# KTH-RPL/HiMo

Measured on AMD Instinct MI355X. Metric: lidar_frames_per_sec_120k, higher is better.
Workload: dtype f16x2 (two-term split fp16, x = h + l with exact subnormals, on the matrix cores; float32 accumulate; ~22-bit products); 1 GPU; per-frame pipeline: pillarise 3 sweeps (512x512 grid) -> SeFlow++-style encoder/decoder + GRU head (random-init, self-specified: reference network source absent) -> per-point flow -> ego-motion removal + dt0 + flow2compDis -> comp_dis; points_per_frame=120000, sweeps_per_frame=3, parallelism=frames sharded x1, refined_output=False, batches_in_flight=3, matrix_arithmetic=f16x2, samples_per_backbone_launch=16, collectives=none (single process)

## Files before the change

himo_amd/csrc/conv_common.h:

```cpp
#pragma once
#include "himo_common.h"
#include "bf16x3.h"
#include <math.h>

namespace himo {

typedef float floatx16 __attribute__((ext_vector_type(16)));

enum Epilogue {
    kEpiBias = 0,
    kEpiBiasBnGelu = 1,
    kEpiBiasGelu = 2,
    kEpiGruZR = 3,
    kEpiGruQ = 4,
    kEpiBiasRelu = 5,
    kEpiReluMask = 6
};

struct ConvArgs {
    const float* x; int64_t x_batch_stride; int x_pitch;
    const float* w;
    const float* bias; const float* scale; const float* shift;
    float* y; int64_t y_batch_stride; int y_pitch;
    int N, H, W, Cin, Cout;
    int n_inner; int64_t x_outer_stride, y_outer_stride;
    int Ho, Wo;
    const float* aux_in; int aux_in_pitch;
    float* aux_out; int aux_out_pitch;
    int act_flags;
    unsigned* range_seen;
    const unsigned long long* mask;
    int64_t mask_batch_stride, mask_outer_stride;
};
enum ActFlags { kActSplitIn = 1, kActSplitOut = 2, kActVecStore = 4, kActAccumulate = 8, kActStuffedIn = 16, kActRowMask = 32 };

__device__ inline int64_t image_offset(int img, int n_inner, int64_t batch_stride, int64_t outer_stride) {
    return (int64_t)(img % n_inner) * batch_stride + (int64_t)(img / n_inner) * outer_stride;
}

__device__ inline int xcd_block_id(int bid, int n_blocks) {
    const int per = n_blocks >> 3, rem = n_blocks & 7;
    const int xcd = bid & 7, idx = bid >> 3;
    return xcd * per + (xcd < rem ? xcd : rem) + idx;
}

__device__ inline float gelu_exact(float v) {
    const float hv = 0.5f * v;
    const float t = __builtin_amdgcn_rcpf(fmaf(0.3275911f * 0.70710678118654752440f, fabsf(v), 1.0f));
    float p = fmaf(1.061405429f, t, -1.453152027f);
    p = fmaf(p, t, 1.421413741f);
    p = fmaf(p, t, -0.284496736f);
    p = fmaf(p, t, 0.254829592f);
    const float ex = __builtin_amdgcn_exp2f((v * v) * (-0.5f * 1.44269504088896340736f));
    const float e = fmaf(-(p * t), ex, 1.0f);
    return fmaf(fabsf(hv), e, hv);
}
__device__ inline float gelu_grad_exact(float v) {
    const float t = __builtin_amdgcn_rcpf(fmaf(0.3275911f * 0.70710678118654752440f, fabsf(v), 1.0f));
    float p = fmaf(1.061405429f, t, -1.453152027f);
    p = fmaf(p, t, 1.421413741f);
    p = fmaf(p, t, -0.284496736f);
    p = fmaf(p, t, 0.254829592f);
    const float ex = __builtin_amdgcn_exp2f((v * v) * (-0.5f * 1.44269504088896340736f));
    const float e = fmaf(-(p * t), ex, 1.0f);
    return fmaf(v * 0.39894228040143267794f, ex, 0.5f + copysignf(0.5f * e, v));
}
__device__ inline float sigmoid_f(float v) { return __builtin_amdgcn_rcpf(1.0f + __expf(-v)); }
__device__ inline float tanh_f(float v) {
    const float e = __expf(-2.0f * fabsf(v));
    const float t = (1.0f - e) * __builtin_amdgcn_rcpf(1.0f + e);
    return copysignf(t, v);
}


template <int EPI> constexpr bool kEpiAffine = EPI == kEpiBias || EPI == kEpiBiasBnGelu || EPI == kEpiBiasGelu;
template <int EPI>
__device__ inline void epi_affine(float k, float bias, float sc, float sh, float& A, float& B) {
    if (EPI == kEpiBiasBnGelu) { A = k * sc; B = fmaf(bias, sc, sh); } else { A = k; B = bias; }
}
template <int EPI>
__device__ inline float epi_activate(float acc, float A, float B) {
    const float v = fmaf(acc, A, B);
    return EPI == kEpiBias ? v : gelu_exact(v);
}

template <int EPI>
__device__ inline void epilogue_store(const ConvArgs& a, float* __restrict__ yout, int64_t pix, int co, float v, float sc, float sh) {
    if (EPI == kEpiBias) {
        yout[pix * a.y_pitch + co] = v;
    } else if (EPI == kEpiBiasBnGelu) {
        v = v * sc + sh;
        yout[pix * a.y_pitch + co] = gelu_exact(v);
    } else if (EPI == kEpiBiasGelu) {
        yout[pix * a.y_pitch + co] = gelu_exact(v);
    } else if (EPI == kEpiGruZR) {
        const int half = a.Cout / 2;
        const float g = sigmoid_f(v);
        if (co < half) yout[pix * a.y_pitch + co] = g;
        else a.aux_out[pix * a.aux_out_pitch + (co - half)] = g * a.aux_in[pix * a.aux_in_pitch + (co - half)];
    } else if (EPI == kEpiBiasRelu) {
        yout[pix * a.y_pitch + co] = fmaxf(v, 0.f);
    } else if (EPI == kEpiReluMask) {
        yout[pix * a.y_pitch + co] = a.aux_in[pix * a.aux_in_pitch + co] > 0.f ? v : 0.f;
    } else if (EPI == kEpiGruQ) {
        const float q = tanh_f(v);
        const float z = a.aux_in[pix * a.aux_in_pitch + co];
        const float h = a.aux_out[pix * a.aux_out_pitch + co];
        a.aux_out[pix * a.aux_out_pitch + co] = (1.0f - z) * h + z * q;
    }
}

__device__ inline unsigned split_word(float v, bool odd);
template <int EPI, bool PAIRED>
__device__ inline void split_store(const ConvArgs& a, float* __restrict__ yout, int64_t pix, int co, float v, float sc, float sh) {
    if (EPI == kEpiBiasBnGelu) v = gelu_exact(v * sc + sh);
    else if (EPI == kEpiBiasGelu) v = gelu_exact(v);
    else if (EPI == kEpiBiasRelu) v = fmaxf(v, 0.f);
    if (PAIRED) {
        const bool odd = co & 1;
        unsigned* rec = reinterpret_cast<unsigned*>(yout + pix * a.y_pitch + (co & ~15));
        rec[(odd ? 8 : 0) + ((co & 15) >> 1)] = split_word(v, odd);
        return;
    }
    unsigned h, l;
    split2_rounded(v, h, l);
    {
        unsigned short* rec = reinterpret_cast<unsigned short*>(yout + pix * a.y_pitch + (co & ~15));
        rec[co & 15] = (unsigned short)h;
        rec[16 + (co & 15)] = (unsigned short)l;
    }
}

constexpr float kSplitRangeGuard = 0.015625f;
__device__ inline void note_range(const ConvArgs& a, float v) {
    if (a.range_seen && __ballot(fabsf(v) >= kSplitRangeGuard) != 0ull && (threadIdx.x & 63) == 0 &&
        __hip_atomic_load(a.range_seen, __ATOMIC_RELAXED, __HIP_MEMORY_SCOPE_AGENT) == 0u)
        __hip_atomic_store(a.range_seen, 1u, __ATOMIC_RELAXED, __HIP_MEMORY_SCOPE_AGENT);
}

inline bool vec_store_ok(const ConvArgs& a) {
    return (reinterpret_cast<uintptr_t>(a.y) & 15u) == 0 && !(a.y_pitch & 3) && !(a.y_batch_stride & 3) && !(a.y_outer_stride & 3) && !(a.Cout & 3) &&
           (int64_t)a.Ho * a.Wo * a.y_pitch < ((int64_t)1 << 29);
}

template <bool OSPLIT, bool MASK = false, bool ACC = false>
__device__ inline void store_block_vec(const ConvArgs& a, float* __restrict__ yout, unsigned char* stg, const unsigned (&word)[16],
                                       int lane, int64_t pix0, int n_valid_px, int ch0) {
    const int li = lane & 31, lh = lane >> 5;
    const int widx = OSPLIT ? (li >> 4) * 16 + ((li & 1) ? 8 : 0) + ((li & 15) >> 1) : li;
#pragma unroll
    for (int r = 0; r < 16; ++r) {
        const int px = (r & 3) + 8 * (r >> 2) + 4 * lh;
        const int slot = px ^ ((px >> 2) & 1);
        *reinterpret_cast<unsigned*>(stg + slot * 128 + widx * 4) = word[r];
    }
    __builtin_amdgcn_wave_barrier();
#pragma unroll
    for (int t = 0; t < 4; ++t) {
        const int q = t * 64 + lane;
        const int slot = q >> 3, piece = q & 7;
        const int px = slot ^ ((slot >> 2) & 1);
        uint4 d = *reinterpret_cast<const uint4*>(stg + q * 16);
        const int ch = ch0 + (OSPLIT ? (piece >> 2) * 16 : piece * 4);
        if (px < n_valid_px && ch < a.Cout) {
            if (MASK) {
                const float4 m = *reinterpret_cast<const float4*>(a.aux_in + (pix0 + px) * (int64_t)a.aux_in_pitch + ch0 + piece * 4);
                d.x = m.x > 0.f ? d.x : 0u; d.y = m.y > 0.f ? d.y : 0u; d.z = m.z > 0.f ? d.z : 0u; d.w = m.w > 0.f ? d.w : 0u;
            }
            float* dst = yout + (((unsigned)pix0 + (unsigned)px) * (unsigned)a.y_pitch + (unsigned)(ch0 + piece * 4));
            if (ACC) {
                const float4 o = *reinterpret_cast<const float4*>(dst);
                d.x = __builtin_bit_cast(unsigned, o.x + __builtin_bit_cast(float, d.x)); d.y = __builtin_bit_cast(unsigned, o.y + __builtin_bit_cast(float, d.y));
                d.z = __builtin_bit_cast(unsigned, o.z + __builtin_bit_cast(float, d.z)); d.w = __builtin_bit_cast(unsigned, o.w + __builtin_bit_cast(float, d.w));
            }
            *reinterpret_cast<uint4*>(dst) = d;
        }
    }
    __builtin_amdgcn_wave_barrier();
}

template <int EPI>
__device__ inline float epilogue_value(float v, float sc, float sh) {
    if (EPI == kEpiBiasBnGelu) return gelu_exact(v * sc + sh);
    if (EPI == kEpiBiasGelu) return gelu_exact(v);
    if (EPI == kEpiBiasRelu) return fmaxf(v, 0.f);
    return v;
}
__device__ inline unsigned split_word(float v, bool odd) {
    const unsigned p = split2_packed(v);
    const unsigned q = (unsigned)__builtin_amdgcn_mov_dpp((int)p, 0xB1, 0xF, 0xF, true);
    return __builtin_amdgcn_perm(q, p, odd ? 0x03020706u : 0x05040100u);
}

}
```

himo_amd/csrc/gruhead.hip:

```cpp
#include "conv_common.h"
#include "bf16x3.h"

namespace himo {

struct GruHeadArgs {
    int64_t n;
    const int* pid; const float* offsets;
    const float* img0; const float* img1; int img_pitch;
    const float* dec; int dec_pitch;
    const float* w_off; const float* b_off;
    const unsigned short* wzr; const float* bzr;
    const unsigned short* wq; const float* bq;
    const unsigned short* w1; const float* b1;
    const float* w2; const float* b2;
    const float* xyz_t; const float* pts; int stride;
    float* flow;
    int iters;
    int img_split;
    unsigned* nonfinite;
    int w2_pitch;
};

constexpr int kGhMaxIters = 4;
struct GruHeadSave {
    float* hx;
    float* rhx;
    float* z; float* r; float* q;
    float* pre1; float* y1;
    float* res;
    int64_t rows;
};

constexpr int kGhMaxSamples = 16;
struct GruHeadSample {
    int64_t n;
    const int* pid; const float* offsets; const float* img0; const float* img1; const float* dec;
    const float* xyz_t; const float* pts; float* flow; int stride;
};
struct GruHeadBatch {
    int n_samples;
    int block_start[kGhMaxSamples + 1];
    GruHeadSample s[kGhMaxSamples];
};

constexpr int kGhRows = 64;
constexpr bool kGhLaunder = false;

template <int SLABS>
__device__ inline int a_slot(int s, int slab, int row, int half) {
    return ((s * SLABS + slab) * kGhRows + row) * 32 + ((half ^ ((row >> 4) & 1)) << 4);
}

template <int FMT, int SLABS>
__device__ inline void a_store(unsigned char* A, int row, int k, float v) {
    constexpr int kGhPlane = SLABS * kGhRows * 32;
    unsigned h, m = 0, l;
    if (FMT == 3) split3(v, h, m, l); else split2(v, h, l);
    const int slab = k >> 4, kk = k & 15;
    const int off = a_slot<SLABS>(0, slab, row, kk >> 3) + (kk & 7) * 2;
    *reinterpret_cast<unsigned short*>(A + off) = (unsigned short)h;
    if (FMT == 3) *reinterpret_cast<unsigned short*>(A + off + kGhPlane) = (unsigned short)m;
    *reinterpret_cast<unsigned short*>(A + off + (FMT - 1) * kGhPlane) = (unsigned short)l;
}

template <int RT, int NT, int FMT, int SLABS>
__device__ inline void gemm192(const unsigned char* A, const unsigned short* __restrict__ wpk, int cout, const int (&col)[NT],
                               floatx16 (&acc)[RT][NT], int rt0, int li, int lh) {
    uint4 bcur[NT][FMT], bnxt[NT][FMT];
    auto load_b = [&](int slab, uint4 (&b)[NT][FMT]) {
#pragma unroll
        for (int t = 0; t < NT; ++t)
#pragma unroll
            for (int s = 0; s < FMT; ++s)
                b[t][s] = *reinterpret_cast<const uint4*>(wpk + (((int64_t)slab * FMT + s) * cout + col[t] + li) * 16 + lh * 8);
    };
    load_b(0, bcur);
    constexpr int kUnroll = SLABS % 2 == 0 ? 2 : 3;
#pragma unroll kUnroll
    for (int slab = 0; slab < SLABS; ++slab) {
        if (slab + 1 < SLABS) load_b(slab + 1, bnxt);
        bf16x8 af[RT][FMT];
#pragma unroll
        for (int rt = 0; rt < RT; ++rt)
#pragma unroll
            for (int s = 0; s < FMT; ++s)
                af[rt][s] = *reinterpret_cast<const bf16x8*>(A + a_slot<SLABS>(s, slab, (rt0 + rt) * 32 + li, lh));
#define HIMO_TERM(SA, SB)                                                                                          \
    _Pragma("unroll") for (int rt = 0; rt < RT; ++rt) _Pragma("unroll") for (int t = 0; t < NT; ++t)                  \
        acc[rt][t] = __builtin_amdgcn_mfma_f32_32x32x16_bf16(af[rt][SA], __builtin_bit_cast(bf16x8, bcur[t][SB]), acc[rt][t], 0, 0, 0);
#define HIMO_TERM16(ACC, SA, SB)                                                                                   \
    _Pragma("unroll") for (int rt = 0; rt < RT; ++rt) _Pragma("unroll") for (int t = 0; t < NT; ++t)                  \
        ACC[rt][t] = __builtin_amdgcn_mfma_f32_32x32x16_f16(__builtin_bit_cast(f16x8, af[rt][SA]),                    \
                                                           __builtin_bit_cast(f16x8, bcur[t][SB]), ACC[rt][t], 0, 0, 0);
        if constexpr (FMT == 3) {
            HIMO_TERM(2, 0) HIMO_TERM(0, 2) HIMO_TERM(1, 1) HIMO_TERM(1, 0) HIMO_TERM(0, 1) HIMO_TERM(0, 0)
        } else {
            HIMO_TERM16(acc, 1, 0) HIMO_TERM16(acc, 0, 1) HIMO_TERM16(acc, 0, 0)
        }
#undef HIMO_TERM16
#undef HIMO_TERM
#pragma unroll
        for (int t = 0; t < NT; ++t)
#pragma unroll
            for (int s = 0; s < FMT; ++s) bcur[t][s] = bnxt[t][s];
    }
    if (FMT == 2) {
#pragma unroll
        for (int rt = 0; rt < RT; ++rt)
#pragma unroll
            for (int t = 0; t < NT; ++t)
#pragma unroll
                for (int r = 0; r < 16; ++r)
                    acc[rt][t][r] = acc[rt][t][r] * kF16AccScale;
    }
}

template <int GROUP>
__device__ inline void sv_store(float* base, unsigned byte_off, float v) {
    *reinterpret_cast<float*>(reinterpret_cast<char*>(base) + byte_off) = v;
}

template <int FMT, int SLABS, bool SAVE = false>
__global__ __launch_bounds__(256, (FMT == 2 && !SAVE) ? 3 : 2) void gru_head_kernel(GruHeadArgs a, GruHeadBatch batch, GruHeadSave sv) {
    constexpr bool FOLD = SLABS == 9;
    static_assert(!(SAVE && FOLD), "the training forward keeps x explicit");
    constexpr int kGhPlane = SLABS * kGhRows * 32;
    __shared__ __attribute__((aligned(16))) unsigned char A[FMT * kGhPlane];
    __shared__ int s_pid[kGhRows];
    const int wave = __builtin_amdgcn_readfirstlane(threadIdx.x >> 6), lane = threadIdx.x & 63;
    const int li = lane & 31, lh = lane >> 5;
    int bid = blockIdx.x;
    {
        int smp = 0;
        while (smp + 1 < batch.n_samples && bid >= batch.block_start[smp + 1]) ++smp;
        bid -= batch.block_start[smp];
        const GruHeadSample& g = batch.s[smp];
        a.n = g.n; a.pid = g.pid; a.offsets = g.offsets; a.img0 = g.img0; a.img1 = g.img1; a.dec = g.dec;
        a.xyz_t = g.xyz_t; a.pts = g.pts; a.flow = g.flow; a.stride = g.stride;
    }
    const int64_t r0 = (int64_t)bid * kGhRows;

    if (threadIdx.x < kGhRows) {
        const int64_t i = r0 + threadIdx.x;
        s_pid[threadIdx.x] = i < a.n ? a.pid[i] : -1;
    }
    if constexpr (FOLD) {
        const int row = threadIdx.x >> 2, q = threadIdx.x & 3;
        const int64_t i = r0 + row;
        float v[4] = {0.f, 0.f, 0.f, 0.f};
        if (q == 0) {
            if (i < a.n) { v[0] = a.offsets[i * 3]; v[1] = a.offsets[i * 3 + 1]; v[2] = a.offsets[i * 3 + 2]; }
            v[3] = 1.f;
        }
#pragma unroll
        for (int k = 0; k < 4; ++k) a_store<FMT, SLABS>(A, row, 128 + q * 4 + k, v[k]);
    } else if constexpr (SAVE) {
        const int c = threadIdx.x & 63;
        const float w0 = a.w_off[c], w1 = a.w_off[64 + c], w2 = a.w_off[128 + c], bc = a.b_off[c];
#pragma unroll 4
        for (int j = 0; j < 16; ++j) {
            const int row = wave + 4 * j;
            const int64_t i = r0 + row;
            const int64_t ic = i < a.n ? i : a.n - 1;
            const float o0 = a.offsets[ic * 3], o1 = a.offsets[ic * 3 + 1], o2 = a.offsets[ic * 3 + 2];
            const float v = fmaf(o2, w2, fmaf(o1, w1, o0 * w0)) + bc;
            a_store<FMT, SLABS>(A, row, 128 + c, v);
            const unsigned at = ((unsigned)i * 192u + 128u + (unsigned)c) * 4u;
            for (int t = 0; t <= a.iters; ++t) sv_store<0>(sv.hx + t * sv.rows * 192, at, v);
            for (int t = 0; t < a.iters; ++t) sv_store<0>(sv.rhx + t * sv.rows * 192, at, v);
        }
    } else {
        const int row = threadIdx.x >> 2, q = threadIdx.x & 3;
        const int64_t i = r0 + row;
        float o0 = 0.f, o1 = 0.f, o2 = 0.f;
        if (i < a.n) { o0 = a.offsets[i * 3]; o1 = a.offsets[i * 3 + 1]; o2 = a.offsets[i * 3 + 2]; }
#pragma unroll
        for (int k = 0; k < 16; ++k) {
            const int c = q * 16 + k;
            const float v = fmaf(o2, a.w_off[128 + c], fmaf(o1, a.w_off[64 + c], o0 * a.w_off[c])) + a.b_off[c];
            a_store<FMT, SLABS>(A, row, 128 + c, v);
        }
    }
    __syncthreads();

    const float* src = wave == 0 ? a.img0 : wave == 1 ? a.img1 : a.dec + (wave - 2) * 32;
    const int src_pitch = wave < 2 ? a.img_pitch : a.dec_pitch;
    float h[2][16];
    {
        int cell[2][16];
#pragma unroll
        for (int rt = 0; rt < 2; ++rt)
#pragma unroll
            for (int r = 0; r < 16; ++r) cell[rt][r] = s_pid[rt * 32 + (r & 3) + 8 * (r >> 2) + 4 * lh];
        if (FMT == 2 && wave < 2 && a.img_split) {
            unsigned short hh[2][16], ll[2][16];
#pragma unroll
            for (int rt = 0; rt < 2; ++rt)
#pragma unroll
                for (int r = 0; r < 16; ++r) {
                    const unsigned short* rec = reinterpret_cast<const unsigned short*>(src + (int64_t)max(cell[rt][r], 0) * src_pitch + (li & ~15));
                    hh[rt][r] = rec[li & 15]; ll[rt][r] = rec[16 + (li & 15)];
                }
#pragma unroll
            for (int rt = 0; rt < 2; ++rt)
#pragma unroll
                for (int r = 0; r < 16; ++r)
                    h[rt][r] = cell[rt][r] >= 0 ? (float)__builtin_bit_cast(_Float16, hh[rt][r]) + (float)__builtin_bit_cast(_Float16, ll[rt][r]) : 0.f;
        } else {
#pragma unroll
            for (int rt = 0; rt < 2; ++rt)
#pragma unroll
                for (int r = 0; r < 16; ++r) h[rt][r] = src[(int64_t)max(cell[rt][r], 0) * src_pitch + li];
#pragma unroll
            for (int rt = 0; rt < 2; ++rt)
#pragma unroll
                for (int r = 0; r < 16; ++r) h[rt][r] = cell[rt][r] >= 0 ? h[rt][r] : 0.f;
            if (FMT == 2 && wave < 2) {
#pragma unroll
                for (int rt = 0; rt < 2; ++rt)
#pragma unroll
                    for (int r = 0; r < 16; ++r) {
                        unsigned hh, ll;
                        split2(h[rt][r], hh, ll);
                        h[rt][r] = (float)__builtin_bit_cast(_Float16, (unsigned short)hh) + (float)__builtin_bit_cast(_Float16, (unsigned short)ll);
                    }
            }
        }
#pragma unroll
        for (int rt = 0; rt < 2; ++rt)
#pragma unroll
            for (int r = 0; r < 16; ++r) {
                const int row = rt * 32 + (r & 3) + 8 * (r >> 2) + 4 * lh;
                a_store<FMT, SLABS>(A, row, wave * 32 + li, h[rt][r]);
                if constexpr (SAVE) sv_store<1>(sv.hx, (((unsigned)r0 + row) * 192u + wave * 32 + li) * 4u, h[rt][r]);
            }
    }
    __syncthreads();
    unsigned o128 = (((unsigned)r0 + 4 * lh) * 128u + wave * 32 + li) * 4u, o192 = (((unsigned)r0 + 4 * lh) * 192u + wave * 32 + li) * 4u;

    const int col_zr[2] = {wave * 32, 128 + wave * 32};
    const int col_q[1] = {wave * 32};
    const float bz = a.bzr[wave * 32 + li], br = a.bzr[128 + wave * 32 + li], bq = a.bq[wave * 32 + li];

#pragma unroll 1
    for (int it = 0; it < a.iters; ++it) {
        int sli = li, slh = lh;
        if constexpr (SAVE || kGhLaunder) asm volatile("" : "+v"(o128), "+v"(o192), "+v"(sli), "+v"(slh));
        float* const sz = SAVE ? sv.z + it * sv.rows * 128 : nullptr; float* const sr = SAVE ? sv.r + it * sv.rows * 128 : nullptr;
        float* const sq = SAVE ? sv.q + it * sv.rows * 128 : nullptr; float* const srhx = SAVE ? sv.rhx + it * sv.rows * 192 : nullptr;
        float* const shx = SAVE ? sv.hx + (it + 1) * sv.rows * 192 : nullptr;
        floatx16 acc[2][2];
#pragma unroll
        for (int rt = 0; rt < 2; ++rt)
#pragma unroll
            for (int t = 0; t < 2; ++t)
#pragma unroll
                for (int r = 0; r < 16; ++r) acc[rt][t][r] = 0.f;
        gemm192<2, 2, FMT, SLABS>(A, a.wzr, 256, col_zr, acc, 0, li, lh);
        __syncthreads();
#pragma unroll
        for (int rt = 0; rt < 2; ++rt)
#pragma unroll
            for (int r = 0; r < 16; ++r) {
                acc[rt][0][r] = sigmoid_f(acc[rt][0][r] + bz);
                const float rr = sigmoid_f(acc[rt][1][r] + br);
                const int row = rt * 32 + (r & 3) + 8 * (r >> 2) + 4 * slh;
                a_store<FMT, SLABS>(A, row, wave * 32 + sli, rr * h[rt][r]);
                if constexpr (SAVE) {
                    const unsigned dr = rt * 32 + (r & 3) + 8 * (r >> 2);
                    sv_store<2>(sz, o128 + dr * 512u, acc[rt][0][r]); sv_store<2>(sr, o128 + dr * 512u, rr);
                    sv_store<3>(srhx, o192 + dr * 768u, rr * h[rt][r]);
                }
            }
        __syncthreads();
        if constexpr (SAVE || kGhLaunder) asm volatile("" : "+v"(o128), "+v"(o192), "+v"(sli), "+v"(slh));
        floatx16 acq[2][1];
#pragma unroll
        for (int rt = 0; rt < 2; ++rt)
#pragma unroll
            for (int r = 0; r < 16; ++r) acq[rt][0][r] = 0.f;
        gemm192<2, 1, FMT, SLABS>(A, a.wq, 128, col_q, acq, 0, li, lh);
        __syncthreads();
#pragma unroll
        for (int rt = 0; rt < 2; ++rt)
#pragma unroll
            for (int r = 0; r < 16; ++r) {
                const float q = tanh_f(acq[rt][0][r] + bq);
                const float zz = acc[rt][0][r];
                const float hn = (1.0f - zz) * h[rt][r] + zz * q;
                h[rt][r] = hn;
                const int row = rt * 32 + (r & 3) + 8 * (r >> 2) + 4 * slh;
                a_store<FMT, SLABS>(A, row, wave * 32 + sli, hn);
                if constexpr (SAVE) {
                    const unsigned dr = rt * 32 + (r & 3) + 8 * (r >> 2);
                    sv_store<4>(sq, o128 + dr * 512u, q);
                    sv_store<5>(shx, o192 + dr * 768u, hn);
                }
            }
        __syncthreads();
    }

    floatx16 ac1[1][1];
#pragma unroll
    for (int r = 0; r < 16; ++r) ac1[0][0][r] = 0.f;
    const int col_1[1] = {0};
    if (wave < 2) gemm192<1, 1, FMT, SLABS>(A, a.w1, 32, col_1, ac1, wave, li, lh);
    __syncthreads();
    float* Y = reinterpret_cast<float*>(A);
    if (wave < 2) {
        const float b1 = a.b1[li];
#pragma unroll
        for (int r = 0; r < 16; ++r) {
            const int row = wave * 32 + (r & 3) + 8 * (r >> 2) + 4 * lh;
            const float pre = ac1[0][0][r] + b1, y = gelu_exact(pre);
            Y[row * 32 + li] = y;
            if constexpr (SAVE) {
                const unsigned at = (((unsigned)r0 + row) * 32u + li) * 4u;
                sv_store<6>(sv.pre1, at, pre); sv_store<6>(sv.y1, at, y);
            }
        }
    }
    __syncthreads();
    if constexpr (SAVE) {
        const int row = threadIdx.x >> 2, c = threadIdx.x & 3;
        const int64_t i = r0 + row;
        float out = 0.f;
        if (c < 3 && s_pid[row] >= 0) {
            const float* y = Y + row * 32;
            float s = y[0] * a.w2[c];
#pragma unroll
            for (int k = 1; k < 32; ++k) s = fmaf(y[k], a.w2[k * a.w2_pitch + c], s);
            out = s + a.b2[c];
        }
        sv.res[i * 4 + c] = out;
        if (a.nonfinite && !(fabsf(out) <= 3.4028234664e38f)) atomicOr(a.nonfinite, 1u);
        return;
    }
    if (threadIdx.x < 3 * kGhRows) {
        const int row = threadIdx.x / 3, c = threadIdx.x % 3;
        const int64_t i = r0 + row;
        if (i < a.n) {
            const float pose_flow = a.xyz_t[i * 3 + c] - a.pts[i * a.stride + c];
            float out = pose_flow;
            if (s_pid[row] >= 0) {
                const float* y = Y + row * 32;
                float s = y[0] * a.w2[c];
#pragma unroll
                for (int k = 1; k < 32; ++k) s = fmaf(y[k], a.w2[k * a.w2_pitch + c], s);
                out = pose_flow + (s + a.b2[c]);
            }
            a.flow[i * 3 + c] = out;
            if (a.nonfinite && !(fabsf(out) <= 3.4028234664e38f)) atomicOr(a.nonfinite, 1u);
        }
    }
}

}

using namespace himo;

static int gru_head_launch(int n_samples, const himo_head_sample* h_samples, int img_pitch, int dec_pitch,
                           const float* d_w_off, const float* d_b_off, bool folded,
                           const void* d_wzr_packed, const float* d_bzr, const void* d_wq_packed, const float* d_bq,
                           const void* d_w1_packed, const float* d_b1, const float* d_w2, const float* d_b2,
                           int iters, int packed_format, int img_split, unsigned* d_nonfinite, void* stream) {
    if (img_split && (packed_format != 1 || (img_pitch & 15))) return HIMO_ERR_INVALID_ARGUMENT;
    if (n_samples < 0 || n_samples > kGhMaxSamples || (n_samples && !h_samples)) return HIMO_ERR_INVALID_ARGUMENT;
    if (iters < 0 || !(packed_format == 0 || packed_format == 1) || img_pitch < 32 || dec_pitch < 64) return HIMO_ERR_INVALID_ARGUMENT;
    if ((!folded && (!d_w_off || !d_b_off)) || !d_wzr_packed || !d_bzr || !d_wq_packed || !d_bq || !d_w1_packed || !d_b1 || !d_w2 || !d_b2)
        return HIMO_ERR_INVALID_ARGUMENT;
    if ((reinterpret_cast<uintptr_t>(d_wzr_packed) | reinterpret_cast<uintptr_t>(d_wq_packed) | reinterpret_cast<uintptr_t>(d_w1_packed)) & 15)
        return HIMO_ERR_INVALID_ARGUMENT;
    GruHeadBatch b{};
    int64_t blocks = 0;
    for (int i = 0; i < n_samples; ++i) {
        const himo_head_sample& h = h_samples[i];
        if (h.n < 0 || h.pc_stride < 3) return HIMO_ERR_INVALID_ARGUMENT;
        if (h.n == 0) continue;
        if (!h.d_pid || !h.d_offsets || !h.d_img0 || !h.d_img1 || !h.d_dec || !h.d_xyz_t || !h.d_pts || !h.d_flow) return HIMO_ERR_INVALID_ARGUMENT;
        GruHeadSample& g = b.s[b.n_samples];
        g.n = h.n; g.pid = h.d_pid; g.offsets = h.d_offsets; g.img0 = h.d_img0; g.img1 = h.d_img1; g.dec = h.d_dec;
        g.xyz_t = h.d_xyz_t; g.pts = h.d_pts; g.flow = h.d_flow; g.stride = h.pc_stride;
        b.block_start[b.n_samples] = (int)blocks;
        blocks += (h.n + kGhRows - 1) / kGhRows;
        if (blocks > 0x7fffffff) return HIMO_ERR_INVALID_ARGUMENT;
        b.block_start[++b.n_samples] = (int)blocks;
    }
    if (!blocks) return HIMO_OK;
    GruHeadArgs a{};
    a.img_pitch = img_pitch; a.dec_pitch = dec_pitch; a.w_off = d_w_off; a.b_off = d_b_off;
    a.wzr = (const unsigned short*)d_wzr_packed; a.bzr = d_bzr; a.wq = (const unsigned short*)d_wq_packed; a.bq = d_bq;
    a.w1 = (const unsigned short*)d_w1_packed; a.b1 = d_b1; a.w2 = d_w2; a.b2 = d_b2; a.iters = iters;
    a.img_split = img_split ? 1 : 0;
    a.nonfinite = d_nonfinite;
    a.w2_pitch = 3;
    hipStream_t s = (hipStream_t)stream;
    ProfScope ps("gru_head_kernel", s);
    const dim3 grid((unsigned)blocks);
    const GruHeadSave none{};
    if (folded) {
        if (packed_format == 1) hipLaunchKernelGGL((gru_head_kernel<2, 9>), grid, dim3(256), 0, s, a, b, none);
        else hipLaunchKernelGGL((gru_head_kernel<3, 9>), grid, dim3(256), 0, s, a, b, none);
    } else {
        if (packed_format == 1) hipLaunchKernelGGL((gru_head_kernel<2, 12>), grid, dim3(256), 0, s, a, b, none);
        else hipLaunchKernelGGL((gru_head_kernel<3, 12>), grid, dim3(256), 0, s, a, b, none);
    }
    HIMO_LAUNCH_CHECK("gru_head_kernel");
    return HIMO_OK;
}

extern "C" int himo_gru_head_batch(int n_samples, const himo_head_sample* h_samples, int img_pitch, int dec_pitch,
                                   const float* d_w_off, const float* d_b_off,
                                   const void* d_wzr_packed, const float* d_bzr, const void* d_wq_packed, const float* d_bq,
                                   const void* d_w1_packed, const float* d_b1, const float* d_w2, const float* d_b2,
                                   int iters, int packed_format, int img_split, void* stream) {
    return gru_head_launch(n_samples, h_samples, img_pitch, dec_pitch, d_w_off, d_b_off, false, d_wzr_packed, d_bzr, d_wq_packed, d_bq,
                           d_w1_packed, d_b1, d_w2, d_b2, iters, packed_format, img_split, nullptr, stream);
}

extern "C" int himo_gru_head_batch_folded(int n_samples, const himo_head_sample* h_samples, int img_pitch, int dec_pitch,
                                          const void* d_wzr_packed, const float* d_bzr, const void* d_wq_packed, const float* d_bq,
                                          const void* d_w1_packed, const float* d_b1, const float* d_w2, const float* d_b2,
                                          int iters, int packed_format, int img_split, void* stream) {
    return gru_head_launch(n_samples, h_samples, img_pitch, dec_pitch, nullptr, nullptr, true, d_wzr_packed, d_bzr, d_wq_packed, d_bq,
                           d_w1_packed, d_b1, d_w2, d_b2, iters, packed_format, img_split, nullptr, stream);
}

extern "C" int himo_gru_head_batch_guarded(int n_samples, const himo_head_sample* h_samples, int img_pitch, int dec_pitch,
                                           const float* d_w_off, const float* d_b_off,
                                           const void* d_wzr_packed, const float* d_bzr, const void* d_wq_packed, const float* d_bq,
                                           const void* d_w1_packed, const float* d_b1, const float* d_w2, const float* d_b2,
                                           int iters, int packed_format, int img_split, uint32_t* d_nonfinite, void* stream) {
    if ((d_w_off == nullptr) != (d_b_off == nullptr)) return HIMO_ERR_INVALID_ARGUMENT;
    return gru_head_launch(n_samples, h_samples, img_pitch, dec_pitch, d_w_off, d_b_off, d_w_off == nullptr, d_wzr_packed, d_bzr, d_wq_packed,
                           d_bq, d_w1_packed, d_b1, d_w2, d_b2, iters, packed_format, img_split, d_nonfinite, stream);
}

extern "C" int himo_gru_head_train(int64_t n, const int32_t* d_pid, const float* d_offsets, const float* d_img0, const float* d_img1,
                                   int img_pitch, const float* d_dec, int dec_pitch, const float* d_w_off, const float* d_b_off,
                                   const void* d_wzr_packed, const float* d_bzr, const void* d_wq_packed, const float* d_bq,
                                   const void* d_w1_packed, const float* d_b1, const float* d_w2, int w2_pitch, const float* d_b2,
                                   int iters, int packed_format, const himo_head_saved* h_saved, uint32_t* d_nonfinite, void* stream) {
    if (n < 0 || iters < 1 || iters > kGhMaxIters || !(packed_format == 0 || packed_format == 1) || img_pitch < 32 || dec_pitch < 64 ||
        !(w2_pitch == 3 || w2_pitch == 4) || !h_saved)
        return HIMO_ERR_INVALID_ARGUMENT;
    if (!d_w_off || !d_b_off || !d_wzr_packed || !d_bzr || !d_wq_packed || !d_bq || !d_w1_packed || !d_b1 || !d_w2 || !d_b2)
        return HIMO_ERR_INVALID_ARGUMENT;
    if ((reinterpret_cast<uintptr_t>(d_wzr_packed) | reinterpret_cast<uintptr_t>(d_wq_packed) | reinterpret_cast<uintptr_t>(d_w1_packed)) & 15)
        return HIMO_ERR_INVALID_ARGUMENT;
    if (n == 0) return HIMO_OK;
    if (!d_pid || !d_offsets || !d_img0 || !d_img1 || !d_dec) return HIMO_ERR_INVALID_ARGUMENT;
    if (h_saved && h_saved->rows * 768 >= ((int64_t)1 << 32)) return HIMO_ERR_UNSUPPORTED;
    GruHeadSave sv{};
    sv.hx = h_saved->d_hx; sv.rhx = h_saved->d_rhx; sv.z = h_saved->d_z; sv.r = h_saved->d_r; sv.q = h_saved->d_q;
    sv.pre1 = h_saved->d_pre1; sv.y1 = h_saved->d_y1; sv.res = h_saved->d_res;
    sv.rows = h_saved->rows;
    if (!sv.hx || !sv.rhx || !sv.z || !sv.r || !sv.q || !sv.pre1 || !sv.y1 || !sv.res || sv.rows < (n + 63) / 64 * 64 || (sv.rows & 63))
        return HIMO_ERR_INVALID_ARGUMENT;
    GruHeadBatch b{};
    b.n_samples = 1;
    GruHeadSample& g = b.s[0];
    g.n = n; g.pid = d_pid; g.offsets = d_offsets; g.img0 = d_img0; g.img1 = d_img1; g.dec = d_dec;
    const int64_t blocks = (n + kGhRows - 1) / kGhRows;
    if (blocks > 0x7fffffff) return HIMO_ERR_INVALID_ARGUMENT;
    b.block_start[0] = 0; b.block_start[1] = (int)blocks;
    GruHeadArgs a{};
    a.img_pitch = img_pitch; a.dec_pitch = dec_pitch; a.w_off = d_w_off; a.b_off = d_b_off;
    a.wzr = (const unsigned short*)d_wzr_packed; a.bzr = d_bzr; a.wq = (const unsigned short*)d_wq_packed; a.bq = d_bq;
    a.w1 = (const unsigned short*)d_w1_packed; a.b1 = d_b1; a.w2 = d_w2; a.b2 = d_b2; a.iters = iters; a.w2_pitch = w2_pitch;
    a.nonfinite = d_nonfinite;
    hipStream_t s = (hipStream_t)stream;
    ProfScope ps("gru_head_train_kernel", s);
    if (packed_format == 1) hipLaunchKernelGGL((gru_head_kernel<2, 12, true>), dim3((unsigned)blocks), dim3(256), 0, s, a, b, sv);
    else hipLaunchKernelGGL((gru_head_kernel<3, 12, true>), dim3((unsigned)blocks), dim3(256), 0, s, a, b, sv);
    HIMO_LAUNCH_CHECK("gru_head_kernel<train>");
    return HIMO_OK;
}

extern "C" int himo_clear_u32(uint32_t* d_words, int n, void* stream) {
    if (!d_words || n < 1) return HIMO_ERR_INVALID_ARGUMENT;
    HIMO_HIP(hipMemsetAsync(d_words, 0, (size_t)n * 4, (hipStream_t)stream));
    return HIMO_OK;
}

extern "C" int himo_gru_head(int64_t n, const int32_t* d_pid, const float* d_offsets, const float* d_img0, const float* d_img1,
                             int img_pitch, const float* d_dec, int dec_pitch, const float* d_w_off, const float* d_b_off,
                             const void* d_wzr_packed, const float* d_bzr, const void* d_wq_packed, const float* d_bq,
                             const void* d_w1_packed, const float* d_b1, const float* d_w2, const float* d_b2,
                             const float* d_xyz_t, const float* d_pts, int pc_stride, float* d_flow, int iters, int packed_format,
                             void* stream) {
    himo_head_sample h{n, d_pid, d_offsets, d_img0, d_img1, d_dec, d_xyz_t, d_pts, pc_stride, d_flow};
    return himo_gru_head_batch(1, &h, img_pitch, dec_pitch, d_w_off, d_b_off, d_wzr_packed, d_bzr, d_wq_packed, d_bq,
                               d_w1_packed, d_b1, d_w2, d_b2, iters, packed_format, 0, stream);
}
```

Baseline: 773.7 frames/s.

## Pack GRU head offset slab and fold gate scale into exp2 FMA

For the fp16-split folded GRU head, the last K slab (the 3 offsets plus a bias-one term) is packed into a single MFMA with a duplicated, compact weight load instead of the three-term split product. The f16 accumulator scale and log2e are folded into one FMA feeding exp2-based sigmoid and tanh, which removes the separate scaling pass in the GEMM. Gate outputs are split into hi/lo f16 with an inline mixed-precision FMA, and a direct single-exp tanh form is used. The packed slab may lose precision on the offset terms, and the new tanh formula behaves differently near saturation.

```diff
diff --git a/himo_amd/csrc/conv_common.h b/himo_amd/csrc/conv_common.h
--- a/himo_amd/csrc/conv_common.h
+++ b/himo_amd/csrc/conv_common.h
@@ -71,6 +71,14 @@
     const float t = (1.0f - e) * __builtin_amdgcn_rcpf(1.0f + e);
     return copysignf(t, v);
 }
+constexpr float kLog2e = 1.44269504088896340736f;
+__device__ inline float sigmoid_from_arg(float x) { return __builtin_amdgcn_rcpf(1.0f + __builtin_amdgcn_exp2f(x)); }
+__device__ inline float tanh_from_arg(float y) {
+    const float e = __builtin_amdgcn_exp2f(-fabsf(y));
+    const float t = (1.0f - e) * __builtin_amdgcn_rcpf(1.0f + e);
+    return copysignf(t, y);
+}
+__device__ inline float tanh_direct_from_arg(float y) { return fmaf(__builtin_amdgcn_rcpf(1.0f + __builtin_amdgcn_exp2f(y)), -2.0f, 1.0f); }
 
 
 template <int EPI> constexpr bool kEpiAffine = EPI == kEpiBias || EPI == kEpiBiasBnGelu || EPI == kEpiBiasGelu;
diff --git a/himo_amd/csrc/gruhead.hip b/himo_amd/csrc/gruhead.hip
--- a/himo_amd/csrc/gruhead.hip
+++ b/himo_amd/csrc/gruhead.hip
@@ -46,6 +46,16 @@
 constexpr int kGhRows = 64;
 constexpr bool kGhLaunder = false;
 
+#ifndef HIMO_HEAD_PACKED_SLAB
+#define HIMO_HEAD_PACKED_SLAB 1
+#endif
+#ifndef HIMO_HEAD_GATE_FMA
+#define HIMO_HEAD_GATE_FMA 1
+#endif
+#ifndef HIMO_HEAD_TANH_DIRECT
+#define HIMO_HEAD_TANH_DIRECT 1
+#endif
+
 template <int SLABS>
 __device__ inline int a_slot(int s, int slab, int row, int half) {
     return ((s * SLABS + slab) * kGhRows + row) * 32 + ((half ^ ((row >> 4) & 1)) << 4);
@@ -63,7 +73,19 @@
     *reinterpret_cast<unsigned short*>(A + off + (FMT - 1) * kGhPlane) = (unsigned short)l;
 }
 
-template <int RT, int NT, int FMT, int SLABS>
+template <int SLABS>
+__device__ inline void a_store_f16(unsigned char* A, int row, int k, float v) {
+    constexpr int kGhPlane = SLABS * kGhRows * 32;
+    const _Float16 hh = (_Float16)v;
+    _Float16 ll;
+    asm("v_fma_mixlo_f16 %0, %1, 1.0, -%2 op_sel_hi:[0,0,1]" : "=v"(ll) : "v"(v), "v"(hh));
+    const int slab = k >> 4, kk = k & 15;
+    const int off = a_slot<SLABS>(0, slab, row, kk >> 3) + (kk & 7) * 2;
+    *reinterpret_cast<_Float16*>(A + off) = hh;
+    *reinterpret_cast<_Float16*>(A + off + kGhPlane) = ll;
+}
+
+template <int RT, int NT, int FMT, int SLABS, bool PK = false, bool SCALE = true>
 __device__ inline void gemm192(const unsigned char* A, const unsigned short* __restrict__ wpk, int cout, const int (&col)[NT],
                                floatx16 (&acc)[RT][NT], int rt0, int li, int lh) {
     uint4 bcur[NT][FMT], bnxt[NT][FMT];
@@ -74,11 +96,68 @@
             for (int s = 0; s < FMT; ++s)
                 b[t][s] = *reinterpret_cast<const uint4*>(wpk + (((int64_t)slab * FMT + s) * cout + col[t] + li) * 16 + lh * 8);
     };
+    static_assert(!PK || FMT == 2, "the packed offset slab is the fp16 split's");
+    constexpr int NFULL = PK ? SLABS - 1 : SLABS;
+    if constexpr (PK) {
+        const unsigned lane_b = (unsigned)(li * 16 + lh * 8) * 2u, lane_p = (unsigned)li * 32u;
+        auto load_bu = [&](int slab, uint4 (&b)[NT][FMT]) {
+            unsigned lane_o = lane_b;
+            asm volatile("" : "+v"(lane_o));
+#pragma unroll
+            for (int t = 0; t < NT; ++t)
+#pragma unroll
+                for (int s = 0; s < FMT; ++s)
+                {
+                    typedef const __attribute__((address_space(1))) char* gptr;
+                    gptr base = (gptr)(reinterpret_cast<const char*>(wpk) + (((int64_t)slab * FMT + s) * cout + col[t]) * 32);
+                    asm volatile("" : "+s"(base));
+                    typedef unsigned u32x4 __attribute__((ext_vector_type(4)));
+                    b[t][s] = __builtin_bit_cast(uint4, *(const __attribute__((address_space(1))) u32x4*)(base + lane_o));
+                }
+        };
+        load_bu(0, bcur);
+#pragma unroll
+        for (int t = 0; t < NT; ++t) {
+            const char* base = reinterpret_cast<const char*>(wpk) + ((int64_t)NFULL * FMT * cout + col[t]) * 32;
+            const uint2 v = *reinterpret_cast<const uint2*>(base + (lh ? (unsigned)cout * 32u + lane_p : lane_p));
+            bnxt[t][0] = uint4{v.x, v.y, v.x, v.y};
+        }
+#pragma unroll
+        for (int rt = 0; rt < RT; ++rt) {
+            const f16x8 af = *reinterpret_cast<const f16x8*>(A + a_slot<SLABS>(0, NFULL, (rt0 + rt) * 32 + li, lh));
+#pragma unroll
+            for (int t = 0; t < NT; ++t)
+                acc[rt][t] = __builtin_amdgcn_mfma_f32_32x32x16_f16(af, __builtin_bit_cast(f16x8, bnxt[t][0]), acc[rt][t], 0, 0, 0);
+        }
+        static_assert(NFULL % 2 == 0, "slab pairs");
+        auto terms = [&](int slab, const uint4 (&b)[NT][FMT]) {
+            f16x8 af[RT][FMT];
+#pragma unroll
+            for (int rt = 0; rt < RT; ++rt)
+#pragma unroll
+                for (int s = 0; s < FMT; ++s)
+                    af[rt][s] = *reinterpret_cast<const f16x8*>(A + a_slot<SLABS>(s, slab, (rt0 + rt) * 32 + li, lh));
+#pragma unroll
+            for (int term = 0; term < 3; ++term)
+#pragma unroll
+                for (int rt = 0; rt < RT; ++rt)
+#pragma unroll
+                    for (int t = 0; t < NT; ++t)
+                        acc[rt][t] = __builtin_amdgcn_mfma_f32_32x32x16_f16(af[rt][term == 0], __builtin_bit_cast(f16x8, b[t][term == 1]), acc[rt][t], 0, 0, 0);
+        };
+#pragma unroll 1
+        for (int slab = 0; slab < NFULL; slab += 2) {
+            load_bu(slab + 1, bnxt);
+            terms(slab, bcur);
+            if (slab + 2 < NFULL) load_bu(slab + 2, bcur);
+            terms(slab + 1, bnxt);
+        }
+    } else {
     load_b(0, bcur);
-    constexpr int kUnroll = SLABS % 2 == 0 ? 2 : 3;
+    constexpr int kUnroll = NFULL % 2 == 0 ? 2 : 3;
 #pragma unroll kUnroll
-    for (int slab = 0; slab < SLABS; ++slab) {
-        if (slab + 1 < SLABS) load_b(slab + 1, bnxt);
+    for (int slab = 0; slab < NFULL; ++slab) {
+        if (slab + 1 < NFULL) load_b(slab + 1, bnxt);
         bf16x8 af[RT][FMT];
 #pragma unroll
         for (int rt = 0; rt < RT; ++rt)
@@ -104,7 +183,8 @@
 #pragma unroll
             for (int s = 0; s < FMT; ++s) bcur[t][s] = bnxt[t][s];
     }
-    if (FMT == 2) {
+    }
+    if (FMT == 2 && SCALE) {
 #pragma unroll
         for (int rt = 0; rt < RT; ++rt)
 #pragma unroll
@@ -124,6 +204,8 @@
 __global__ __launch_bounds__(256, (FMT == 2 && !SAVE) ? 3 : 2) void gru_head_kernel(GruHeadArgs a, GruHeadBatch batch, GruHeadSave sv) {
     constexpr bool FOLD = SLABS == 9;
     static_assert(!(SAVE && FOLD), "the training forward keeps x explicit");
+    constexpr bool DIET = FMT == 2 && FOLD && !SAVE;
+    constexpr bool PKSLAB = DIET && HIMO_HEAD_PACKED_SLAB, GFMA = DIET && HIMO_HEAD_GATE_FMA;
     constexpr int kGhPlane = SLABS * kGhRows * 32;
     __shared__ __attribute__((aligned(16))) unsigned char A[FMT * kGhPlane];
     __shared__ int s_pid[kGhRows];
@@ -144,7 +226,20 @@
         const int64_t i = r0 + threadIdx.x;
         s_pid[threadIdx.x] = i < a.n ? a.pid[i] : -1;
     }
-    if constexpr (FOLD) {
+    if constexpr (PKSLAB) {
+        const int row = threadIdx.x >> 2, q = threadIdx.x & 3;
+        const int64_t i = r0 + row;
+        float v[4] = {0.f, 0.f, 0.f, 1.f};
+        if (i < a.n) { v[0] = a.offsets[i * 3]; v[1] = a.offsets[i * 3 + 1]; v[2] = a.offsets[i * 3 + 2]; }
+        unsigned w[4];
+#pragma unroll
+        for (int k = 0; k < 4; ++k) {
+            unsigned hh, ll;
+            split2(v[k], hh, ll);
+            w[k] = q == 3 ? 0u : q == 1 ? ll : hh;
+        }
+        *reinterpret_cast<uint2*>(A + a_slot<SLABS>(0, 8, row, q >> 1) + (q & 1) * 8) = uint2{w[0] | (w[1] << 16), w[2] | (w[3] << 16)};
+    } else if constexpr (FOLD) {
         const int row = threadIdx.x >> 2, q = threadIdx.x & 3;
         const int64_t i = r0 + row;
         float v[4] = {0.f, 0.f, 0.f, 0.f};
@@ -256,16 +351,24 @@
             for (int t = 0; t < 2; ++t)
 #pragma unroll
                 for (int r = 0; r < 16; ++r) acc[rt][t][r] = 0.f;
-        gemm192<2, 2, FMT, SLABS>(A, a.wzr, 256, col_zr, acc, 0, li, lh);
+        gemm192<2, 2, FMT, SLABS, PKSLAB, !GFMA>(A, a.wzr, 256, col_zr, acc, 0, li, lh);
         __syncthreads();
+        const float kAs = -kLog2e * kF16AccScale, kBz = -kLog2e * bz, kBr = -kLog2e * br;
 #pragma unroll
         for (int rt = 0; rt < 2; ++rt)
 #pragma unroll
             for (int r = 0; r < 16; ++r) {
-                acc[rt][0][r] = sigmoid_f(acc[rt][0][r] + bz);
-                const float rr = sigmoid_f(acc[rt][1][r] + br);
+                float rr;
+                if constexpr (GFMA) {
+                    acc[rt][0][r] = sigmoid_from_arg(fmaf(acc[rt][0][r], kAs, kBz));
+                    rr = sigmoid_from_arg(fmaf(acc[rt][1][r], kAs, kBr));
+                } else {
+                    acc[rt][0][r] = sigmoid_f(acc[rt][0][r] + bz);
+                    rr = sigmoid_f(acc[rt][1][r] + br);
+                }
                 const int row = rt * 32 + (r & 3) + 8 * (r >> 2) + 4 * slh;
-                a_store<FMT, SLABS>(A, row, wave * 32 + sli, rr * h[rt][r]);
+                if constexpr (GFMA) a_store_f16<SLABS>(A, row, wave * 32 + sli, rr * h[rt][r]);
+                else a_store<FMT, SLABS>(A, row, wave * 32 + sli, rr * h[rt][r]);
                 if constexpr (SAVE) {
                     const unsigned dr = rt * 32 + (r & 3) + 8 * (r >> 2);
                     sv_store<2>(sz, o128 + dr * 512u, acc[rt][0][r]); sv_store<2>(sr, o128 + dr * 512u, rr);
@@ -279,18 +382,26 @@
         for (int rt = 0; rt < 2; ++rt)
 #pragma unroll
             for (int r = 0; r < 16; ++r) acq[rt][0][r] = 0.f;
-        gemm192<2, 1, FMT, SLABS>(A, a.wq, 128, col_q, acq, 0, li, lh);
+        gemm192<2, 1, FMT, SLABS, PKSLAB, !GFMA>(A, a.wq, 128, col_q, acq, 0, li, lh);
         __syncthreads();
+        const float kAt = 2.0f * kLog2e * kF16AccScale, kBq = 2.0f * kLog2e * bq;
 #pragma unroll
         for (int rt = 0; rt < 2; ++rt)
 #pragma unroll
             for (int r = 0; r < 16; ++r) {
-                const float q = tanh_f(acq[rt][0][r] + bq);
+                float q;
+                if constexpr (GFMA) {
+                    const float y = fmaf(acq[rt][0][r], kAt, kBq);
+                    if constexpr (HIMO_HEAD_TANH_DIRECT) q = tanh_direct_from_arg(y); else q = tanh_from_arg(y);
+                } else {
+                    q = tanh_f(acq[rt][0][r] + bq);
+                }
                 const float zz = acc[rt][0][r];
                 const float hn = (1.0f - zz) * h[rt][r] + zz * q;
                 h[rt][r] = hn;
                 const int row = rt * 32 + (r & 3) + 8 * (r >> 2) + 4 * slh;
-                a_store<FMT, SLABS>(A, row, wave * 32 + sli, hn);
+                if constexpr (GFMA) a_store_f16<SLABS>(A, row, wave * 32 + sli, hn);
+                else a_store<FMT, SLABS>(A, row, wave * 32 + sli, hn);
                 if constexpr (SAVE) {
                     const unsigned dr = rt * 32 + (r & 3) + 8 * (r >> 2);
                     sv_store<4>(sq, o128 + dr * 512u, q);
@@ -304,7 +415,7 @@
 #pragma unroll
     for (int r = 0; r < 16; ++r) ac1[0][0][r] = 0.f;
     const int col_1[1] = {0};
-    if (wave < 2) gemm192<1, 1, FMT, SLABS>(A, a.w1, 32, col_1, ac1, wave, li, lh);
+    if (wave < 2) gemm192<1, 1, FMT, SLABS, PKSLAB>(A, a.w1, 32, col_1, ac1, wave, li, lh);
     __syncthreads();
     float* Y = reinterpret_cast<float*>(A);
     if (wave < 2) {
```

Result: faster. 788.0 frames/s (median of 6 runs) (+1.9%).
